# ai4co/rl4co

Hardware: AMD Instinct MI355X
Metric: decode_steps_per_sec (higher is better)
Workload: dtype bf16; 1 GPU; BASELINE configs[1]: TSPEnv num_loc=100 batch=4096/GPU AttentionModel(3L,d128,h8) greedy rollout, bf16 encoder GEMMs, bf16 cache; leg=c2_greedy, batch_per_gpu=4096, cache_dtype=bf16, launch=pipeline, input=one synthetic batch resident in HBM, reused by every step, parallelism=replicas x1 (instances sharded)

## Files before the change

### rl4co_amd/csrc/am_decode.hip

```cpp
#include <hip/hip_runtime.h>

#include "common.h"
#include "rl4co_math.h"

namespace {

constexpr int kD = RL4CO_EMBED_DIM;
constexpr int kH = RL4CO_NUM_HEADS;
constexpr int kDH = kD / kH;
constexpr int kUnroll = 4;
constexpr float kNegInf = -__builtin_huge_valf();
constexpr float kSqrtD = 11.3137084989847604f;

struct CacheF32 {
  using elem = float;
  using raw = float4;
  static constexpr int EPL = 4;
  __device__ static inline raw zero() { return make_float4(0.f, 0.f, 0.f, 0.f); }
  __device__ static inline raw ld(const elem* p) { return *reinterpret_cast<const float4*>(p); }
  __device__ static inline void cvt(const raw& t, float (&v)[4]) {
    v[0] = t.x; v[1] = t.y; v[2] = t.z; v[3] = t.w;
  }
};

// ... 146 lines not shown
      key = rl4co_expf(lp) / nz;
    }
    if (bc == 0x7fffffff || key > best) {
      best = key;
      bc = c;
    }
    if (a.entropy && lp > kNegInf) ent = fmaf(rl4co_expf(lp), lp, ent);
    if (alp) alp[j] = lp;
  }
  rl4co::bfly_argmax(best, bc);
  if (a.entropy) st.ent_acc = st.ent_acc - rl4co::bfly_sum<1, 64>(ent);
  wave_lds_sync();
  return commit_and_step<ENV>(a, st, lg, fl, F, mk, vis, dem, cap, r, t, N, lane, oplocs, opmax, twdur, bc);
}

template <int ENV>
__device__ inline int commit_and_step(const rl4co_am_decode_args& a, TrajState& st, float* lg, const uint16_t* fl, int F,
                                      uint8_t* mk, uint8_t* vis, const float* dem, float cap, int r, int t, int N, int lane,
                                      const float* oplocs, const float* opmax, const float* twdur, int bc) {
  const int64_t tcol = (int64_t)a.t0 + t;
  int bi;
  float logp;
  if (a.mode == RL4CO_DECODE_EVALUATE) {
    bi = (int)a.forced_actions[(int64_t)r * a.out_stride + tcol];
    if (bi < 0 || bi >= N) {
      st.errbits |= RL4CO_EBIT_INFEASIBLE;
      bi = 0;
    }
    int pos = 0x7fffffff;
    for (int c = lane; c < F; c += 64)
      if (fl[c] == bi) pos = c;
    pos = -rl4co::bfly_i_max(-pos);
    logp = pos < F ? lg[pos] : kNegInf;
  } else {
    bi = (bc < F) ? (int)fl[bc] : 0;
    logp = (bc < F) ? lg[bc] : kNegInf;
  }
  if (mk[bi] == 0) st.errbits |= RL4CO_EBIT_INFEASIBLE;
  if (!(logp > -1000.0f)) st.errbits |= RL4CO_EBIT_NEG_INF_LOGP;
  if (lane == 0) {
    a.actions[(int64_t)r * a.out_stride + tcol] = bi;
    a.logps[(int64_t)r * a.out_stride + tcol] = logp;
  }
  wave_lds_sync();

  if (ENV == RL4CO_ENV_TSP) {
    if (st.step_i == 0) st.first = bi;
    st.cur = bi;
    if (lane == 0) mk[bi] = 0;
    st.step_i += 1;
    wave_lds_sync();
    bool any_left = false;
    for (int j = lane; j < N; j += 64) any_left |= mk[j] != 0;
    st.done = !__any(any_left);
  } else if (ENV == RL4CO_ENV_PDP) {
    const int n = N - 1;
    if (lane == 0) {
      vis[bi] &= (uint8_t)~1u;
      vis[(bi + n / 2) % (n + 1)] |= 2;
    }
    st.step_i += 1;
    st.cur = bi;
    wave_lds_sync();
    bool left = false;
    for (int j = lane; j < N; j += 64) {
      const uint8_t v = vis[j];
      mk[j] = (v == 3) ? 1 : 0;
      left |= (v & 1) != 0;
    }
    st.done = !__any(left);
  } else if (ENV == RL4CO_ENV_PCTSP) {
    st.used = st.used + dem[bi];
    if (lane == 0) vis[bi] = 1;
    st.done = (bi == 0) && (st.step_i > 0);
    st.step_i += 1;
    st.cur = bi;
    wave_lds_sync();
    const bool depot_visited = vis[0] != 0;
    bool unvisited = false;
    for (int j = lane; j < N; j += 64) {
      if (j >= 1) {
        mk[j] = (vis[j] != 0 || depot_visited) ? 0 : 1;
        unvisited |= vis[j] == 0;
      }
    }
    unvisited = __any(unvisited);
    if (lane == 0) mk[0] = ((st.used < 1.0f) && unvisited) ? 0 : 1;
  } else if (ENV == RL4CO_ENV_OP) {
    const float cx = oplocs[2 * st.cur], cy = oplocs[2 * st.cur + 1];
    const float bx = oplocs[2 * bi], by = oplocs[2 * bi + 1];
    {
      const float dx = bx - cx, dy = by - cy;
      st.used = st.used + sqrtf(fmaf(dy, dy, dx * dx));
    }
    if (lane == 0) vis[bi] = 1;
    st.done = (bi == 0) && (st.step_i > 0);
    st.step_i += 1;
    st.cur = bi;
    wave_lds_sync();
    const bool depot_visited = vis[0] != 0;
    for (int j = lane; j < N; j += 64) {
      const float dx = oplocs[2 * j] - bx, dy = oplocs[2 * j + 1] - by;
      const bool exceeds = st.used + sqrtf(fmaf(dy, dy, dx * dx)) > opmax[j];
      mk[j] = (j == 0 || !(vis[j] != 0 || depot_visited || exceeds)) ? 1 : 0;
    }
  } else {
    if (ENV == RL4CO_ENV_CVRPTW) {
      const float dx = oplocs[2 * bi] - oplocs[2 * st.cur], dy = oplocs[2 * bi + 1] - oplocs[2 * st.cur + 1];
      const float served = fmaxf(st.time + sqrtf(fmaf(dy, dy, dx * dx)), opmax[2 * bi]) + twdur[bi];
      st.time = (bi != 0 ? 1.0f : 0.0f) * served;
    }
    const int di = min(max(bi - 1, 0), N - 2);
    st.used = (st.used + dem[di]) * (bi != 0 ? 1.0f : 0.0f);
    st.cur = bi;
    if (lane == 0) vis[bi] = 1;
    wave_lds_sync();
    const float thr = cap + 1e-5f;
    bool any_feasible = false, all_visited = true;
    for (int j = lane; j < N; j += 64) {
      all_visited &= vis[j] != 0;
      if (j >= 1) {
        const bool masked = (vis[j] != 0) || (dem[j - 1] + st.used > thr);
        mk[j] = masked ? 0 : 1;
        any_feasible |= !masked;
      }
    }
    any_feasible = __any(any_feasible);
    st.done = __all(all_visited);
    if (lane == 0) mk[0] = ((st.cur == 0) && any_feasible) ? 0 : 1;
    if (ENV == RL4CO_ENV_CVRPTW) {
      wave_lds_sync();
      const float bx = oplocs[2 * bi], by = oplocs[2 * bi + 1];
      for (int j = lane; j < N; j += 64) {
        const float dx = oplocs[2 * j] - bx, dy = oplocs[2 * j + 1] - by;
        if (!(st.time + sqrtf(fmaf(dy, dy, dx * dx)) <= opmax[2 * j + 1])) mk[j] = 0;
      }
    }
  }
  wave_lds_sync();
  return bi;
}

template <int EPL>
__device__ inline void gemv_t(float (&out)[EPL], const float* __restrict__ wt, const float* in_lds, int width, int e0) {
#pragma unroll
  for (int e = 0; e < EPL; ++e) out[e] = 0.0f;
  for (int k = 0; k < width; ++k) {
    const float c = in_lds[k];
#pragma unroll
    for (int e = 0; e < EPL; ++e) out[e] = fmaf(wt[(int64_t)k * kD + e0 + e], c, out[e]);
  }
}

template <class C, int ENV, bool UNFOLD = false>
__global__ void __launch_bounds__(64) am_decode_kernel(const rl4co_am_decode_args a) {
  constexpr int EPL = C::EPL;
  constexpr int LPR = kD / EPL;
  constexpr int RPL = 64 / LPR;
  constexpr int LPH = kDH / EPL;
  using elem = typename C::elem;
  using raw_t = typename C::raw;

  extern __shared__ __align__(16) unsigned char smem[];
  const int lane = threadIdx.x;
  const int r = trajectory_of_block(blockIdx.x, a.B, a.B_inst);
  const int N = a.N;
  const int Np = lds_pad(N);
  float* sc = reinterpret_cast<float*>(smem);
  float* lg = sc + Np * kH;
  float* mh = lg + Np;
  uint16_t* fl = reinterpret_cast<uint16_t*>(mh + kH);
  uint8_t* mk = reinterpret_cast<uint8_t*>(fl + Np);
  uint8_t* vis = mk + Np;

  const int cb = r % a.B_inst;
  const int rg = lane / LPR;
  const int li = lane % LPR;
  const int hd = li / LPH;
  const int e0 = li * EPL;

  const elem* Kg = static_cast<const elem*>(a.glimpse_key) + (int64_t)cb * a.kvl_batch_stride + e0;
  const elem* Vg = static_cast<const elem*>(a.glimpse_val) + (int64_t)cb * a.kvl_batch_stride + e0;
  const elem* Kl = static_cast<const elem*>(a.logit_key) + (int64_t)cb * a.kvl_batch_stride + e0;
  const int64_t rs = a.kvl_row_stride;
  const CtxTables<C> ctx(a, cb, N, e0);
  const float* hrow = UNFOLD ? a.node_embed + (int64_t)cb * N * kD + e0 : nullptr;

  uint8_t* gmask = a.action_mask + (int64_t)r * N;
  for (int j = lane; j < Np; j += 64) mk[j] = (j < N) ? gmask[j] : (uint8_t)0;
  constexpr bool kScalarCtx = ENV == RL4CO_ENV_CVRP || ENV == RL4CO_ENV_OP || ENV == RL4CO_ENV_PCTSP || ENV == RL4CO_ENV_CVRPTW;
  constexpr bool kCvrpLike = ENV == RL4CO_ENV_CVRP || ENV == RL4CO_ENV_CVRPTW;
  if (ENV == RL4CO_ENV_PDP) {
    const uint8_t* gv = a.visited + (int64_t)r * N;
    const uint8_t* gt = a.to_deliver + (int64_t)r * N;
    for (int j = lane; j < Np; j += 64) vis[j] = (j < N) ? (uint8_t)((gv[j] != 0 ? 1 : 0) | (gt[j] != 0 ? 2 : 0)) : (uint8_t)0;
  } else if (ENV != RL4CO_ENV_TSP) {
    const uint8_t* gv = a.visited + (int64_t)r * N;
    for (int j = lane; j < Np; j += 64) vis[j] = (j < N) ? gv[j] : (uint8_t)1;
  }
  TrajState st;
  st.cur = (int)a.current_node[r];
  st.first = (ENV == RL4CO_ENV_TSP) ? (int)a.first_node[r] : 0;
  st.step_i = !kCvrpLike ? a.step_i[r] : 0;
  st.time = (ENV == RL4CO_ENV_CVRPTW) ? a.current_time[r] : 0.0f;
  st.used = kScalarCtx ? a.used_capacity[r] : 0.0f;
  st.done = a.done[r] != 0;
  st.errbits = 0;
  st.ent_acc = 0.0f;
  const float* oplocs = (ENV == RL4CO_ENV_OP || ENV == RL4CO_ENV_CVRPTW) ? a.locs + (int64_t)cb * N * 2 : nullptr;
  const float* opmax = (ENV == RL4CO_ENV_OP)       ? a.max_length + (int64_t)cb * N
                       : (ENV == RL4CO_ENV_CVRPTW) ? a.time_windows + (int64_t)cb * N * 2
                                                   : nullptr;
  const float* twdur = (ENV == RL4CO_ENV_CVRPTW) ? a.durations + (int64_t)cb * N : nullptr;
  const float cap = (kCvrpLike || ENV == RL4CO_ENV_PCTSP) ? a.vehicle_capacity[r]
                                                                      : ((ENV == RL4CO_ENV_OP) ? opmax[0] : 0.0f);
  const float* dem = kCvrpLike                  ? a.demand + (int64_t)cb * (N - 1)
                     : (ENV == RL4CO_ENV_PCTSP) ? a.demand + (int64_t)cb * N
                                                : nullptr;
  wave_lds_sync();

  float qb[EPL];
#pragma unroll
  for (int e = 0; e < EPL; ++e) qb[e] = a.q_bias ? a.q_bias[(int64_t)cb * kD + e0 + e] : 0.0f;

  const bool single = a.max_steps == 1;
  int t = 0;
  int rows_read = 0;

  for (; t < a.max_steps && (!st.done || single); ++t) {
    const int F = build_list(a, mk, fl, N, lane);
    rows_read += F;

    float q[EPL];
    if constexpr (UNFOLD) {
      float* cv = sc;
      if (rg == 0) {
        if (ENV == RL4CO_ENV_TSP) {
          const bool ph = st.step_i < 1;
#pragma unroll
          for (int e = 0; e < EPL; ++e) {
            cv[e0 + e] = ph ? a.w_placeholder[e0 + e] : hrow[(int64_t)st.first * kD + e];
            cv[kD + e0 + e] = ph ? a.w_placeholder[kD + e0 + e] : hrow[(int64_t)st.cur * kD + e];
          }
        } else {
#pragma unroll
          for (int e = 0; e < EPL; ++e) cv[e0 + e] = hrow[(int64_t)st.cur * kD + e];
          if (li == 0) cv[kD] = cap - st.used;
        }
      }
      wave_lds_sync();
      gemv_t<EPL>(q, a.w_ctx_t, cv, a.ctx_width, e0);
#pragma unroll
      for (int e = 0; e < EPL; ++e) q[e] = q[e] + qb[e];
      wave_lds_sync();
    } else if (ENV == RL4CO_ENV_TSP) {
      if (st.step_i < 1) {
#pragma unroll
        for (int e = 0; e < EPL; ++e) q[e] = a.q_step0[e0 + e] + qb[e];
      } else {
        float cf[EPL], cc[EPL];
        ctx.load(ctx.first, st.first, cf);
        ctx.load(ctx.cur, st.cur, cc);
#pragma unroll
        for (int e = 0; e < EPL; ++e) q[e] = (cf[e] + cc[e]) + qb[e];
      }
    } else if (ENV == RL4CO_ENV_PDP) {
      float cc[EPL];
      ctx.load(ctx.cur, st.cur, cc);
#pragma unroll
      for (int e = 0; e < EPL; ++e) q[e] = cc[e] + qb[e];
    } else {
      float rem = cap - st.used;
      if (ENV == RL4CO_ENV_PCTSP && !(rem > 0.0f)) rem = 0.0f;
      float cc[EPL];
      ctx.load(ctx.cur, st.cur, cc);
#pragma unroll
      for (int e = 0; e < EPL; ++e) {
        float v = fmaf(a.w_cap[e0 + e], rem, cc[e]);
        if (ENV == RL4CO_ENV_CVRPTW) v = fmaf(a.w_time[e0 + e], st.time, v);
        q[e] = v + qb[e];
      }
    }
#pragma unroll
    for (int e = 0; e < EPL; ++e) q[e] = q[e] * 0.25f;

    float m = kNegInf;
    for (int c0 = 0; c0 < F; c0 += RPL * kUnroll) {
      raw_t rw[kUnroll];
      int jj[kUnroll];
#pragma unroll
      for (int u = 0; u < kUnroll; ++u) {
        const int c = c0 + u * RPL + rg;
        jj[u] = (c < F) ? (int)fl[c] : -1;
        rw[u] = (jj[u] >= 0) ? C::ld(Kg + (int64_t)jj[u] * rs) : C::zero();
      }
#pragma unroll
      for (int u = 0; u < kUnroll; ++u) {
        const int c = c0 + u * RPL + rg;
        const bool valid = jj[u] >= 0;
        float k[EPL];
        C::cvt(rw[u], k);
        float acc = 0.0f;
#pragma unroll
        for (int e = 0; e < EPL; ++e) acc = fmaf(q[e], k[e], acc);
        acc = rl4co::bfly_sum<1, LPH>(acc);
        const bool feas = valid && (!a.mask_inner || mk[valid ? jj[u] : 0] != 0);
        const float sv = feas ? acc : kNegInf;
        if (valid && (li % LPH) == 0) sc[c * kH + hd] = sv;
        m = fmaxf(m, sv);
      }
    }
    m = rl4co::bfly_max<LPR, 64>(m);
    if (rg == 0 && (li % LPH) == 0) mh[hd] = m;
    wave_lds_sync();
    {
      const float mm = mh[lane & (kH - 1)];
      for (int idx = lane; idx < F * kH; idx += 64) sc[idx] = rl4co_expf(sc[idx] - mm);
    }
    wave_lds_sync();

    float l = 0.0f;
    float o[EPL];
#pragma unroll
    for (int e = 0; e < EPL; ++e) o[e] = 0.0f;
    for (int c0 = 0; c0 < F; c0 += RPL * kUnroll) {
      raw_t rw[kUnroll];
      bool ok[kUnroll];
#pragma unroll
      for (int u = 0; u < kUnroll; ++u) {
        const int c = c0 + u * RPL + rg;
        ok[u] = c < F;
        rw[u] = ok[u] ? C::ld(Vg + (int64_t)fl[c] * rs) : C::zero();
      }
#pragma unroll
      for (int u = 0; u < kUnroll; ++u) {
        const int c = c0 + u * RPL + rg;
        float v[EPL];
        C::cvt(rw[u], v);
        const float p = ok[u] ? sc[c * kH + hd] : 0.0f;
        l = l + p;
#pragma unroll
        for (int e = 0; e < EPL; ++e) o[e] = fmaf(p, v[e], o[e]);
      }
    }
    l = 1.0f / rl4co::bfly_sum<LPR, 64>(l);
#pragma unroll
    for (int e = 0; e < EPL; ++e) o[e] = rl4co::bfly_sum<LPR, 64>(o[e]) * l;
    if constexpr (UNFOLD) {
      wave_lds_sync();
      if (rg == 0) {
#pragma unroll
        for (int e = 0; e < EPL; ++e) sc[e0 + e] = o[e];
      }
      wave_lds_sync();
      gemv_t<EPL>(o, a.w_out_t, sc, kD, e0);
    }

    for (int c0 = 0; c0 < F; c0 += RPL * kUnroll) {
      raw_t rw[kUnroll];
#pragma unroll
      for (int u = 0; u < kUnroll; ++u) {
        const int c = c0 + u * RPL + rg;
        rw[u] = (c < F) ? C::ld(Kl + (int64_t)fl[c] * rs) : C::zero();
      }
#pragma unroll
      for (int u = 0; u < kUnroll; ++u) {
        const int c = c0 + u * RPL + rg;
        float k[EPL];
        C::cvt(rw[u], k);
        float acc = 0.0f;
#pragma unroll
        for (int e = 0; e < EPL; ++e) acc = fmaf(o[e], k[e], acc);
        acc = rl4co::bfly_sum<1, LPR>(acc);
        if (c < F && li == 0) lg[c] = acc;
      }
    }
    wave_lds_sync();

    finalize_and_step<ENV>(a, st, lg, fl, F, mk, vis, dem, cap, r, t, N, lane, oplocs, opmax, twdur);
  }
  if (!single && !st.done && t >= a.max_steps) st.errbits |= RL4CO_EBIT_MAX_STEPS;

  for (int j = lane; j < N; j += 64) gmask[j] = mk[j];
  if (ENV == RL4CO_ENV_PDP) {
    uint8_t* gv = a.visited + (int64_t)r * N;
    uint8_t* gt = a.to_deliver + (int64_t)r * N;
    for (int j = lane; j < N; j += 64) {
      gv[j] = vis[j] & 1;
      gt[j] = (vis[j] >> 1) & 1;
    }
  } else if (ENV != RL4CO_ENV_TSP) {
    uint8_t* gv = a.visited + (int64_t)r * N;
    for (int j = lane; j < N; j += 64) gv[j] = vis[j];
  }
  if (lane == 0) {
    a.current_node[r] = st.cur;
    a.done[r] = st.done ? 1 : 0;
    if (ENV == RL4CO_ENV_TSP) a.first_node[r] = st.first;
    if (!kCvrpLike) a.step_i[r] = st.step_i;
    if (ENV == RL4CO_ENV_CVRPTW) a.current_time[r] = st.time;
    if (kScalarCtx) a.used_capacity[r] = st.used;
    if (a.n_steps) a.n_steps[r] = t;
    if (a.steps_summary) {
      atomicMax(a.steps_summary, t);
      atomicAdd(a.steps_summary + 1, t);
      atomicAdd(reinterpret_cast<unsigned long long*>(a.steps_summary + 2), (unsigned long long)rows_read);
    }
    if (a.entropy) a.entropy[r] += st.ent_acc;
    if (st.errbits) atomicOr(a.err, (int)st.errbits);
  }
}

constexpr int kLdsWaves = 4;
constexpr int kLdsGroups = 16;

template <int ENV>
__device__ inline int wide_scores(const rl4co_am_decode_args& a, TrajState& st, float* lg, const uint16_t* fl, int F,
                                  const uint8_t* mk, float* xs, int nw, int r, int t, int N, int tid) {
  constexpr int T = 64 * kLdsWaves;
  const int w = tid >> 6, lane = tid & 63;
  float* ex = xs;
  float* xw = xs + 2 * nw;
  bool nan_seen = false;
  float zmax = kNegInf;
  for (int c = tid; c < F; c += T) {
    float z = lg[c] / kSqrtD;
    if (z != z) nan_seen = true;
    if (a.tanh_clipping > 0.0f) z = rl4co_tanhf(z) * a.tanh_clipping;
    if (a.mask_logits && mk[fl[c]] == 0) z = kNegInf;
    if (a.temperature != 1.0f) z = z / a.temperature;
    lg[c] = z;
    zmax = fmaxf(zmax, z);
  }
  zmax = rl4co::bfly_max<1, 64>(zmax);
  const bool wave_nan = __any(nan_seen);
  if (lane == 0) {
    xw[w] = zmax;
    xw[4 + w] = wave_nan ? 1.0f : 0.0f;
  }
  __syncthreads();
  zmax = fmaxf(fmaxf(xw[0], xw[1]), fmaxf(xw[2], xw[3]));
  if ((xw[4] + xw[5]) + (xw[6] + xw[7]) != 0.0f) st.errbits |= RL4CO_EBIT_NAN_LOGIT;
  for (int c = tid; c < F; c += T) ex[c] = rl4co_expf(lg[c] - zmax);
  __syncthreads();
  if (w == 0) {
    float zsum = 0.0f;
    for (int c = lane; c < F; c += 64) zsum = zsum + ex[c];
    zsum = rl4co::bfly_sum<1, 64>(zsum);
    if (lane == 0) xw[8] = rl4co_logf(zsum);
  }
  __syncthreads();
  const float lse = xw[8];
  const int64_t tcol = (int64_t)a.t0 + t;
  float* alp = a.all_logps ? a.all_logps + ((int64_t)r * a.out_stride + tcol) * N : nullptr;
  if (alp && F < N) {
    for (int j = tid; j < N; j += T)
      if (mk[j] == 0) alp[j] = kNegInf;
  }
  for (int c = tid; c < F; c += T) {
    const int j = fl[c];
    const float lp = (lg[c] - zmax) - lse;
    lg[c] = lp;
    float key = lp;
    if (a.mode == RL4CO_DECODE_SAMPLE) {
      const float nz = a.exp_noise
                           ? a.exp_noise[((int64_t)t * a.B + r) * N + j]
                           : rl4co_exp1_noise(a.philox_seed ^ (a.philox_seed_dev ? *a.philox_seed_dev : 0ull),
                                              a.philox_offset + (uint64_t)tcol, (uint32_t)r,
                                              (uint32_t)j);
      key = rl4co_expf(lp) / nz;
    }
    ex[c] = key;
    if (alp) alp[j] = lp;
  }
  __syncthreads();
  int bc = 0x7fffffff;
  if (w == 0) {
    float best = kNegInf, ent = 0.0f;
    for (int c = lane; c < F; c += 64) {
      const float key = ex[c];
      if (bc == 0x7fffffff || key > best) {
        best = key;
        bc = c;
      }
      if (a.entropy) {
        const float lp = lg[c];
        if (lp > kNegInf) ent = fmaf(rl4co_expf(lp), lp, ent);
      }
    }
    rl4co::bfly_argmax(best, bc);
    if (a.entropy) st.ent_acc = st.ent_acc - rl4co::bfly_sum<1, 64>(ent);
    wave_lds_sync();
  }
  return bc;
}

__host__ __device__ inline int lds_variant_sc_rows(int N) { return N < 80 ? 80 : N; }
__host__ __device__ inline int wide_scratch_bytes(int N) {
  const int nw = (N + 3) & ~3;
  return lds_variant_sc_rows(N) * kH * 4 + nw * 4 + kLdsWaves * kH * 4 + 32 + 2 * nw + 2 * nw;
}
__host__ __device__ inline int lds_variant_bytes(int N) { return 3 * N * kD * 2 + wide_scratch_bytes(N); }

template <int ENV, bool RESIDENT, class C = CacheBF16>
__global__ void __launch_bounds__(64 * kLdsWaves, 4) am_decode_wide_kernel(const rl4co_am_decode_args a) {
  constexpr int EPL = 8, LPR = 16, LPH = 2;
  constexpr int U = 4;
  extern __shared__ __align__(16) unsigned char smem[];
  const int tid = threadIdx.x;
  const int w = tid >> 6, lane = tid & 63;
  const int r = trajectory_of_block(blockIdx.x, a.B, a.B_inst);
  const int N = a.N;
  const int nw = (N + 3) & ~3;
  uint16_t* planes = reinterpret_cast<uint16_t*>(smem);
  float* sc = reinterpret_cast<float*>(planes + (RESIDENT ? 3 * N * kD : 0));
  float* lg = sc + lds_variant_sc_rows(N) * kH;
  float* mpart = lg + nw;
  int* shi = reinterpret_cast<int*>(mpart + kLdsWaves * kH);
  uint16_t* fl = reinterpret_cast<uint16_t*>(shi + 8);
  uint8_t* mk = reinterpret_cast<uint8_t*>(fl + nw);
  uint8_t* vis = mk + nw;

  const int cb = r % a.B_inst;
  const int rg = lane / LPR, li = lane % LPR, hd = li / LPH, e0 = li * EPL;
  const uint16_t *Kg, *Vg, *Kl;
  int64_t rs;
  if constexpr (RESIDENT) {
    Kg = planes + e0;
    Vg = planes + N * kD + e0;
    Kl = planes + 2 * N * kD + e0;
    rs = kD;
  } else {
// ... 148 lines not shown
#pragma unroll
    for (int e = 0; e < EPL; ++e) o[e] = 0.0f;
    for (int i0 = 0; i0 < iters; i0 += U) {
      uint4 rw[U];
      bool ok[U];
#pragma unroll
      for (int u = 0; u < U; ++u) {
        const int c = kLdsGroups * (i0 + u) + 4 * w + rg;
        ok[u] = c < F;
        rw[u] = ok[u] ? *reinterpret_cast<const uint4*>(Vg + (int64_t)fl[c] * rs) : C::zero();
      }
#pragma unroll
      for (int u = 0; u < U; ++u) {
        const int c = kLdsGroups * (i0 + u) + 4 * w + rg;
        float v[EPL];
        C::cvt(rw[u], v);
        const float p = ok[u] ? sc[c * kH + hd] : 0.0f;
        l = l + p;
#pragma unroll
        for (int e = 0; e < EPL; ++e) o[e] = fmaf(p, v[e], o[e]);
      }
    }
    l = rl4co::bfly_sum<LPR, 64>(l);
#pragma unroll
    for (int e = 0; e < EPL; ++e) o[e] = rl4co::bfly_sum<LPR, 64>(o[e]);
    if (rg == 0) {
#pragma unroll
      for (int e = 0; e < EPL; ++e) *opart(w, e0 + e) = o[e];
      if ((li & 1) == 0) *lpart(w, hd) = l;
    }
    __syncthreads();
    l = 1.0f / ((*lpart(0, hd) + *lpart(1, hd)) + (*lpart(2, hd) + *lpart(3, hd)));
#pragma unroll
    for (int e = 0; e < EPL; ++e) {
      const int d = e0 + e;
      o[e] = ((*opart(0, d) + *opart(1, d)) + (*opart(2, d) + *opart(3, d))) * l;
    }

    for (int i0 = 0; i0 < iters; i0 += U) {
      uint4 rw[U];
#pragma unroll
      for (int u = 0; u < U; ++u) {
        const int c = kLdsGroups * (i0 + u) + 4 * w + rg;
        rw[u] = (c < F) ? *reinterpret_cast<const uint4*>(Kl + (int64_t)fl[c] * rs) : C::zero();
      }
#pragma unroll
      for (int u = 0; u < U; ++u) {
        const int c = kLdsGroups * (i0 + u) + 4 * w + rg;
        float k[EPL];
        C::cvt(rw[u], k);
        float acc = 0.0f;
#pragma unroll
        for (int e = 0; e < EPL; ++e) acc = fmaf(o[e], k[e], acc);
        acc = rl4co::bfly_sum<1, LPR>(acc);
        if (c < F && li == 0) lg[c] = acc;
      }
    }
    __syncthreads();

    const int bc = wide_scores<ENV>(a, st, lg, fl, F, mk, sc, nw, r, t, N, tid);
    if (w == 0) {
      commit_and_step<ENV>(a, st, lg, fl, F, mk, vis, dem, cap, r, t, N, lane, oplocs, opmax, twdur, bc);
      const int Fn = build_list(a, mk, fl, N, lane);
      if (lane == 0) {
        shi[0] = st.cur;
        shi[1] = st.done ? 1 : 0;
        shi[2] = Fn;
        shi[3] = st.first;
        shi[4] = (int)st.step_i;
        shi[5] = __float_as_int(st.used);
        shi[6] = __float_as_int(st.time);
      }
    }
    __syncthreads();
    if (w != 0) {
      st.cur = shi[0];
      st.done = shi[1] != 0;
      st.first = shi[3];
      st.step_i = shi[4];
      st.used = __int_as_float(shi[5]);
      st.time = __int_as_float(shi[6]);
    }
  }
  if (w == 0) {
    if (!single && !st.done && t >= a.max_steps) st.errbits |= RL4CO_EBIT_MAX_STEPS;
    for (int j = lane; j < N; j += 64) gmask[j] = mk[j];
    if (ENV == RL4CO_ENV_PDP) {
      uint8_t* gv = a.visited + (int64_t)r * N;
      uint8_t* gt = a.to_deliver + (int64_t)r * N;
      for (int j = lane; j < N; j += 64) {
        gv[j] = vis[j] & 1;
        gt[j] = (vis[j] >> 1) & 1;
      }
    } else if (ENV != RL4CO_ENV_TSP) {
      uint8_t* gv = a.visited + (int64_t)r * N;
      for (int j = lane; j < N; j += 64) gv[j] = vis[j];
    }
    if (lane == 0) {
      a.current_node[r] = st.cur;
      a.done[r] = st.done ? 1 : 0;
      if (ENV == RL4CO_ENV_TSP) a.first_node[r] = st.first;
      if (!kCvrpLike) a.step_i[r] = st.step_i;
      if (ENV == RL4CO_ENV_CVRPTW) a.current_time[r] = st.time;
      if (kScalarCtx) a.used_capacity[r] = st.used;
      if (a.n_steps) a.n_steps[r] = t;
      if (a.steps_summary) {
        atomicMax(a.steps_summary, t);
        atomicAdd(a.steps_summary + 1, t);
        atomicAdd(reinterpret_cast<unsigned long long*>(a.steps_summary + 2), (unsigned long long)(RESIDENT ? 0 : rows_read));
      }
      if (a.entropy) a.entropy[r] += st.ent_acc;
      if (st.errbits) atomicOr(a.err, (int)st.errbits);
    }
  }
}

template <int ENV, bool RESIDENT, class C>
int launch_wide_c(const rl4co_am_decode_args& a, hipStream_t stream) {
  const int lds = RESIDENT ? lds_variant_bytes(a.N) : wide_scratch_bytes(a.N);
  if (lds > 64 * 1024) {
    RL4CO_HIP_TRY(hipFuncSetAttribute(reinterpret_cast<const void*>(am_decode_wide_kernel<ENV, RESIDENT, C>),
                                      hipFuncAttributeMaxDynamicSharedMemorySize, lds));
  }
  hipLaunchKernelGGL((am_decode_wide_kernel<ENV, RESIDENT, C>), dim3(a.B), dim3(64 * kLdsWaves), lds, stream, a);
  RL4CO_HIP_TRY(hipGetLastError());
  return RL4CO_OK;
}
template <int ENV, bool RESIDENT>
int launch_wide(const rl4co_am_decode_args& a, hipStream_t stream) {
  return a.cache_dtype == RL4CO_DT_F16 ? launch_wide_c<ENV, RESIDENT, CacheF16>(a, stream)
                                       : launch_wide_c<ENV, RESIDENT, CacheBF16>(a, stream);
}

inline int resolve_variant(const rl4co_am_decode_args& a) {
  if (a.unfold) return (a.variant == RL4CO_VARIANT_AUTO || a.variant == RL4CO_VARIANT_STREAM) ? RL4CO_VARIANT_STREAM : -1;
  const bool f16 = a.cache_dtype == RL4CO_DT_F16;
  const bool bf16 = a.cache_dtype == RL4CO_DT_BF16 || f16;
  const bool ms_ok = bf16 && a.N <= 128 && a.B_inst > 0 && a.all_logps == nullptr && a.entropy == nullptr;
  if (a.variant == RL4CO_VARIANT_MS) return ms_ok ? RL4CO_VARIANT_MS : -1;
  const bool fits = bf16 && lds_variant_bytes(a.N) <= 80 * 1024;
  const bool wide_ok = bf16 && wide_scratch_bytes(a.N) <= 64 * 1024;
  if (a.variant == RL4CO_VARIANT_STREAM) return RL4CO_VARIANT_STREAM;
  if (a.variant == RL4CO_VARIANT_LDS) return fits ? RL4CO_VARIANT_LDS : -1;
  if (a.variant == RL4CO_VARIANT_WIDE) return wide_ok ? RL4CO_VARIANT_WIDE : -1;
  if (a.max_steps < 4) return RL4CO_VARIANT_STREAM;
  const int ms_from = (a.env == RL4CO_ENV_TSP || a.env == RL4CO_ENV_PDP || a.env == RL4CO_ENV_PCTSP) ? 3
                      : (a.env == RL4CO_ENV_CVRP ? 8 : 0);
  if (ms_ok && ms_from > 0 && a.B >= ms_from * a.B_inst) return RL4CO_VARIANT_MS;
  if (fits && a.B <= 1024) return RL4CO_VARIANT_LDS;
  if (wide_ok && a.B <= 2048) return RL4CO_VARIANT_WIDE;
  return RL4CO_VARIANT_STREAM;
}

template <class C, int ENV, bool UNFOLD = false>
int launch(const rl4co_am_decode_args& a, hipStream_t stream) {
  const int lds = rl4co_am_decode_lds_bytes(a.N, ENV);
  if (lds > 64 * 1024) {
    RL4CO_HIP_TRY(hipFuncSetAttribute(reinterpret_cast<const void*>(am_decode_kernel<C, ENV, UNFOLD>),
                                      hipFuncAttributeMaxDynamicSharedMemorySize, lds));
  }
  hipLaunchKernelGGL((am_decode_kernel<C, ENV, UNFOLD>), dim3(a.B), dim3(64), lds, stream, a);
  RL4CO_HIP_TRY(hipGetLastError());
  return RL4CO_OK;
}

}

extern "C" int rl4co_am_decode_lds_bytes(int N, int env) {
  (void)env;
  const int Np = lds_pad(N);
  return Np * kH * 4 + Np * 4 + kH * 4 + Np * 2 + Np + Np;
}

extern "C" int rl4co_am_decode_row_groups(const rl4co_am_decode_args* args) {
  if (args == nullptr) return -1;
  const int v = resolve_variant(*args);
  if (v < 0) return -1;
  if (v == RL4CO_VARIANT_MS) return 0;
  if (v == RL4CO_VARIANT_LDS || v == RL4CO_VARIANT_WIDE) return kLdsGroups;
  return args->cache_dtype != RL4CO_DT_F32 ? 64 / (kD / CacheBF16::EPL) : 64 / (kD / CacheF32::EPL);
}

extern "C" int rl4co_am_decode_variant(const rl4co_am_decode_args* args) {
  return args == nullptr ? -1 : resolve_variant(*args);
}

extern "C" int rl4co_am_decode(const rl4co_am_decode_args* args, void* stream) {
  RL4CO_REQUIRE(args != nullptr);
  const rl4co_am_decode_args& a = *args;
  RL4CO_REQUIRE(a.env == RL4CO_ENV_TSP || a.env == RL4CO_ENV_CVRP || a.env == RL4CO_ENV_OP ||
                a.env == RL4CO_ENV_PCTSP || a.env == RL4CO_ENV_PDP || a.env == RL4CO_ENV_CVRPTW);
  RL4CO_REQUIRE(a.B > 0 && a.B_inst > 0 && a.B % a.B_inst == 0);
  RL4CO_REQUIRE(a.N >= 2 && a.N <= 4096);
  RL4CO_REQUIRE(a.max_steps >= 1);
  RL4CO_REQUIRE(a.mode >= RL4CO_DECODE_GREEDY && a.mode <= RL4CO_DECODE_EVALUATE);
  RL4CO_REQUIRE(a.cache_dtype == RL4CO_DT_F32 || a.cache_dtype == RL4CO_DT_BF16 || a.cache_dtype == RL4CO_DT_F16);
  RL4CO_REQUIRE(a.cache_dtype != RL4CO_DT_F16 || !a.unfold);
  RL4CO_REQUIRE(a.glimpse_key && a.glimpse_val && a.logit_key && (a.ctx_cur || a.unfold));
  RL4CO_REQUIRE(a.unfold == 0 || a.unfold == 1);
  RL4CO_REQUIRE(a.ctx_dtype == RL4CO_DT_F32 || (a.ctx_dtype == a.cache_dtype && !a.unfold));
  RL4CO_REQUIRE(a.ctx_row_stride == 0 || (a.ctx_row_stride >= kD && a.ctx_row_stride % 8 == 0));
  RL4CO_REQUIRE(a.ctx_batch_stride == 0 || (a.ctx_batch_stride >= (int64_t)a.N * kD && a.ctx_batch_stride % 8 == 0));
  RL4CO_REQUIRE(a.ctx_dtype == RL4CO_DT_F32 || ((reinterpret_cast<uintptr_t>(a.ctx_cur) | reinterpret_cast<uintptr_t>(a.ctx_first)) & 15) == 0);
  if (a.unfold) {
    RL4CO_REQUIRE(a.env == RL4CO_ENV_TSP || a.env == RL4CO_ENV_CVRP);
    RL4CO_REQUIRE(a.node_embed && a.w_ctx_t && a.w_out_t);
    RL4CO_REQUIRE(a.ctx_width == (a.env == RL4CO_ENV_TSP ? 2 * kD : kD + 1));
    RL4CO_REQUIRE(a.env != RL4CO_ENV_TSP || a.w_placeholder);
  }
  RL4CO_REQUIRE(a.kvl_row_stride >= kD && a.kvl_row_stride % 8 == 0);
  RL4CO_REQUIRE(a.kvl_batch_stride >= (int64_t)a.N * kD && a.kvl_batch_stride % 8 == 0);
  RL4CO_REQUIRE(a.action_mask && a.current_node && a.done && a.actions && a.logps && a.err);
  RL4CO_REQUIRE(a.out_stride >= 1 && a.t0 >= 0 && (int64_t)a.t0 + a.max_steps <= a.out_stride);
  RL4CO_REQUIRE(a.temperature > 0.0f);
  RL4CO_REQUIRE((reinterpret_cast<uintptr_t>(a.steps_summary) & 7) == 0);
  RL4CO_REQUIRE(a.mode != RL4CO_DECODE_EVALUATE || a.forced_actions != nullptr);
  if (a.env == RL4CO_ENV_TSP) {
    RL4CO_REQUIRE(((a.ctx_first && a.q_step0) || a.unfold) && a.first_node && a.step_i);
  } else if (a.env == RL4CO_ENV_CVRP) {
    RL4CO_REQUIRE((a.w_cap || a.unfold) && a.demand && a.used_capacity && a.vehicle_capacity && a.visited);
  } else if (a.env == RL4CO_ENV_CVRPTW) {
    RL4CO_REQUIRE(a.w_cap && a.w_time && a.demand && a.used_capacity && a.vehicle_capacity && a.visited);
    RL4CO_REQUIRE(a.locs && a.time_windows && a.durations && a.current_time);
  } else if (a.env == RL4CO_ENV_PDP) {
    RL4CO_REQUIRE(a.visited && a.to_deliver && a.step_i && (a.N - 1) % 2 == 0);
  } else if (a.env == RL4CO_ENV_PCTSP) {
    RL4CO_REQUIRE(a.w_cap && a.demand && a.used_capacity && a.vehicle_capacity && a.step_i && a.visited);
  } else {
    RL4CO_REQUIRE(a.w_cap && a.locs && a.max_length && a.used_capacity && a.step_i && a.visited);
  }
  RL4CO_REQUIRE(rl4co_am_decode_lds_bytes(a.N, a.env) <= 160 * 1024);
  RL4CO_REQUIRE(a.variant >= RL4CO_VARIANT_AUTO && a.variant <= RL4CO_VARIANT_MS);
  const int variant = resolve_variant(a);
  RL4CO_REQUIRE(variant >= 0);
  hipStream_t s = rl4co::as_stream(stream);
  if (a.unfold) {
    if (a.cache_dtype == RL4CO_DT_F32)
      return a.env == RL4CO_ENV_TSP ? launch<CacheF32, RL4CO_ENV_TSP, true>(a, s) : launch<CacheF32, RL4CO_ENV_CVRP, true>(a, s);
    return a.env == RL4CO_ENV_TSP ? launch<CacheBF16, RL4CO_ENV_TSP, true>(a, s) : launch<CacheBF16, RL4CO_ENV_CVRP, true>(a, s);
  }
  if (variant == RL4CO_VARIANT_MS && a.cache_dtype == RL4CO_DT_F16) return rl4co::launch_decode_ms_f16(a, s);
  if (variant == RL4CO_VARIANT_MS) return rl4co::launch_decode_ms(a, s);
  if (variant == RL4CO_VARIANT_LDS || variant == RL4CO_VARIANT_WIDE) {
    const bool res = variant == RL4CO_VARIANT_LDS;
    switch (a.env) {
      case RL4CO_ENV_TSP: return res ? launch_wide<RL4CO_ENV_TSP, true>(a, s) : launch_wide<RL4CO_ENV_TSP, false>(a, s);
      case RL4CO_ENV_CVRP: return res ? launch_wide<RL4CO_ENV_CVRP, true>(a, s) : launch_wide<RL4CO_ENV_CVRP, false>(a, s);
      case RL4CO_ENV_OP: return res ? launch_wide<RL4CO_ENV_OP, true>(a, s) : launch_wide<RL4CO_ENV_OP, false>(a, s);
      case RL4CO_ENV_PCTSP: return res ? launch_wide<RL4CO_ENV_PCTSP, true>(a, s) : launch_wide<RL4CO_ENV_PCTSP, false>(a, s);
      case RL4CO_ENV_PDP: return res ? launch_wide<RL4CO_ENV_PDP, true>(a, s) : launch_wide<RL4CO_ENV_PDP, false>(a, s);
      default: return res ? launch_wide<RL4CO_ENV_CVRPTW, true>(a, s) : launch_wide<RL4CO_ENV_CVRPTW, false>(a, s);
    }
  }
  if (a.cache_dtype == RL4CO_DT_F16) {
    switch (a.env) {
      case RL4CO_ENV_TSP: return launch<CacheF16, RL4CO_ENV_TSP>(a, s);
      case RL4CO_ENV_CVRP: return launch<CacheF16, RL4CO_ENV_CVRP>(a, s);
      case RL4CO_ENV_OP: return launch<CacheF16, RL4CO_ENV_OP>(a, s);
      case RL4CO_ENV_PCTSP: return launch<CacheF16, RL4CO_ENV_PCTSP>(a, s);
      case RL4CO_ENV_PDP: return launch<CacheF16, RL4CO_ENV_PDP>(a, s);
      default: return launch<CacheF16, RL4CO_ENV_CVRPTW>(a, s);
    }
  }
  if (a.env == RL4CO_ENV_CVRPTW)
    return a.cache_dtype == RL4CO_DT_F32 ? launch<CacheF32, RL4CO_ENV_CVRPTW>(a, s)
                                         : launch<CacheBF16, RL4CO_ENV_CVRPTW>(a, s);
  if (a.env == RL4CO_ENV_PDP)
    return a.cache_dtype == RL4CO_DT_F32 ? launch<CacheF32, RL4CO_ENV_PDP>(a, s) : launch<CacheBF16, RL4CO_ENV_PDP>(a, s);
  if (a.env == RL4CO_ENV_PCTSP)
    return a.cache_dtype == RL4CO_DT_F32 ? launch<CacheF32, RL4CO_ENV_PCTSP>(a, s)
                                         : launch<CacheBF16, RL4CO_ENV_PCTSP>(a, s);
  if (a.env == RL4CO_ENV_OP)
    return a.cache_dtype == RL4CO_DT_F32 ? launch<CacheF32, RL4CO_ENV_OP>(a, s) : launch<CacheBF16, RL4CO_ENV_OP>(a, s);
  if (a.cache_dtype == RL4CO_DT_F32) {
    return a.env == RL4CO_ENV_TSP ? launch<CacheF32, RL4CO_ENV_TSP>(a, s)
                                  : launch<CacheF32, RL4CO_ENV_CVRP>(a, s);
  }
  return a.env == RL4CO_ENV_TSP ? launch<CacheBF16, RL4CO_ENV_TSP>(a, s)
                                : launch<CacheBF16, RL4CO_ENV_CVRP>(a, s);
}
```

Before: 131.6 million instance·step/s.

## Software-pipeline K/V/logit-key row loads across decode phases and set waves_per_eu

Restructures the three gather loops in the AM decode kernel so each loop issues the next block's row loads after computing the current block. The first block of the next phase (Kg→Vg→Kl) is loaded while the previous phase is still finishing, and for most envs the first Kg block is issued before the query is built. This hides global-memory latency behind compute and LDS syncs. It also adds an amdgpu_waves_per_eu(4) hint, which can limit registers; the extra live registers from prefetching could raise register pressure or cause spills.

```diff
diff --git a/rl4co_amd/csrc/am_decode.hip b/rl4co_amd/csrc/am_decode.hip
--- a/rl4co_amd/csrc/am_decode.hip
+++ b/rl4co_amd/csrc/am_decode.hip
@@ -323,7 +323,7 @@
 }
 
 template <class C, int ENV, bool UNFOLD = false>
-__global__ void __launch_bounds__(64) am_decode_kernel(const rl4co_am_decode_args a) {
+__global__ void __launch_bounds__(64) __attribute__((amdgpu_waves_per_eu(4))) am_decode_kernel(const rl4co_am_decode_args a) {
   constexpr int EPL = C::EPL;
   constexpr int LPR = kD / EPL;
   constexpr int RPL = 64 / LPR;
@@ -397,9 +397,22 @@
   int t = 0;
   int rows_read = 0;
 
+  constexpr int kBlk = RPL * kUnroll;
+  raw_t rw[kUnroll];
+  int F = 0;
+  auto load_block = [&](const elem* P, int c0) {
+#pragma unroll
+    for (int u = 0; u < kUnroll; ++u) {
+      const int c = c0 + u * RPL + rg;
+      rw[u] = (c < F) ? C::ld(P + (int64_t)fl[c] * rs) : C::zero();
+    }
+  };
+
   for (; t < a.max_steps && (!st.done || single); ++t) {
-    const int F = build_list(a, mk, fl, N, lane);
+    F = build_list(a, mk, fl, N, lane);
     rows_read += F;
+    constexpr bool kAhead = ENV != RL4CO_ENV_OP && ENV != RL4CO_ENV_CVRPTW;
+    if (kAhead) load_block(Kg, 0);
 
     float q[EPL];
     if constexpr (UNFOLD) {
@@ -453,31 +466,30 @@
     }
 #pragma unroll
     for (int e = 0; e < EPL; ++e) q[e] = q[e] * 0.25f;
+    if (!kAhead) load_block(Kg, 0);
 
     float m = kNegInf;
-    for (int c0 = 0; c0 < F; c0 += RPL * kUnroll) {
-      raw_t rw[kUnroll];
-      int jj[kUnroll];
+    for (int c0 = 0; c0 < F; c0 += kBlk) {
 #pragma unroll
       for (int u = 0; u < kUnroll; ++u) {
         const int c = c0 + u * RPL + rg;
-        jj[u] = (c < F) ? (int)fl[c] : -1;
-        rw[u] = (jj[u] >= 0) ? C::ld(Kg + (int64_t)jj[u] * rs) : C::zero();
-      }
-#pragma unroll
-      for (int u = 0; u < kUnroll; ++u) {
-        const int c = c0 + u * RPL + rg;
-        const bool valid = jj[u] >= 0;
+        const bool valid = c < F;
+        const int j = valid ? (int)fl[c] : 0;
         float k[EPL];
         C::cvt(rw[u], k);
         float acc = 0.0f;
 #pragma unroll
         for (int e = 0; e < EPL; ++e) acc = fmaf(q[e], k[e], acc);
         acc = rl4co::bfly_sum<1, LPH>(acc);
-        const bool feas = valid && (!a.mask_inner || mk[valid ? jj[u] : 0] != 0);
+        const bool feas = valid && (!a.mask_inner || mk[j] != 0);
         const float sv = feas ? acc : kNegInf;
         if (valid && (li % LPH) == 0) sc[c * kH + hd] = sv;
         m = fmaxf(m, sv);
+      }
+      if (c0 + kBlk < F) {
+        load_block(Kg, c0 + kBlk);
+      } else if (kAhead) {
+        load_block(Vg, 0);
       }
     }
     m = rl4co::bfly_max<LPR, 64>(m);
@@ -488,29 +500,27 @@
       for (int idx = lane; idx < F * kH; idx += 64) sc[idx] = rl4co_expf(sc[idx] - mm);
     }
     wave_lds_sync();
+    if (!kAhead) load_block(Vg, 0);
 
     float l = 0.0f;
     float o[EPL];
 #pragma unroll
     for (int e = 0; e < EPL; ++e) o[e] = 0.0f;
-    for (int c0 = 0; c0 < F; c0 += RPL * kUnroll) {
-      raw_t rw[kUnroll];
-      bool ok[kUnroll];
-#pragma unroll
-      for (int u = 0; u < kUnroll; ++u) {
-        const int c = c0 + u * RPL + rg;
-        ok[u] = c < F;
-        rw[u] = ok[u] ? C::ld(Vg + (int64_t)fl[c] * rs) : C::zero();
-      }
+    for (int c0 = 0; c0 < F; c0 += kBlk) {
 #pragma unroll
       for (int u = 0; u < kUnroll; ++u) {
         const int c = c0 + u * RPL + rg;
         float v[EPL];
         C::cvt(rw[u], v);
-        const float p = ok[u] ? sc[c * kH + hd] : 0.0f;
+        const float p = (c < F) ? sc[c * kH + hd] : 0.0f;
         l = l + p;
 #pragma unroll
         for (int e = 0; e < EPL; ++e) o[e] = fmaf(p, v[e], o[e]);
+      }
+      if (c0 + kBlk < F) {
+        load_block(Vg, c0 + kBlk);
+      } else if (kAhead && !UNFOLD) {
+        load_block(Kl, 0);
       }
     }
     l = 1.0f / rl4co::bfly_sum<LPR, 64>(l);
@@ -525,14 +535,9 @@
       wave_lds_sync();
       gemv_t<EPL>(o, a.w_out_t, sc, kD, e0);
     }
-
-    for (int c0 = 0; c0 < F; c0 += RPL * kUnroll) {
-      raw_t rw[kUnroll];
-#pragma unroll
-      for (int u = 0; u < kUnroll; ++u) {
-        const int c = c0 + u * RPL + rg;
-        rw[u] = (c < F) ? C::ld(Kl + (int64_t)fl[c] * rs) : C::zero();
-      }
+    if (UNFOLD || !kAhead) load_block(Kl, 0);
+
+    for (int c0 = 0; c0 < F; c0 += kBlk) {
 #pragma unroll
       for (int u = 0; u < kUnroll; ++u) {
         const int c = c0 + u * RPL + rg;
@@ -544,6 +549,7 @@
         acc = rl4co::bfly_sum<1, LPR>(acc);
         if (c < F && li == 0) lg[c] = acc;
       }
+      if (c0 + kBlk < F) load_block(Kl, c0 + kBlk);
     }
     wave_lds_sync();
 
```

After: 131.0 million instance·step/s (median of 2 runs). About the same (-0.5%).

## Cache a few candidate K/V/logit-key rows in spare LDS for the stream decode

Applied to the files above, without the earlier changes.

Adds a small per-workgroup LDS row cache for TSP and CVRP in the stream decode kernel. Cached candidates are taken from the tail of the feasible list. The three cache planes (glimpse key, glimpse value, logit key) are filled on first read, and later steps read from LDS instead of HBM. When a node leaves the candidate set its slot passes to the next candidate. The slot count is sized on the host so it never lowers workgroups per CU. The aim is less HBM gather traffic per step, at the cost of extra per-step bookkeeping, wave reductions and LDS syncs, for what may be only a handful of cached rows.

```diff
diff --git a/rl4co_amd/csrc/am_decode.hip b/rl4co_amd/csrc/am_decode.hip
--- a/rl4co_amd/csrc/am_decode.hip
+++ b/rl4co_amd/csrc/am_decode.hip
@@ -322,12 +322,18 @@
   }
 }
 
+constexpr int kRowCacheNone = 0xFF;
+__host__ __device__ inline int row_cache_bytes(int N, int S, int esz) {
+  return S > 0 ? S * 3 * kD * esz + lds_pad(N) + S : 0;
+}
+
 template <class C, int ENV, bool UNFOLD = false>
-__global__ void __launch_bounds__(64) am_decode_kernel(const rl4co_am_decode_args a) {
+__global__ void __launch_bounds__(64) am_decode_kernel(const rl4co_am_decode_args a, const int S) {
   constexpr int EPL = C::EPL;
   constexpr int LPR = kD / EPL;
   constexpr int RPL = 64 / LPR;
   constexpr int LPH = kDH / EPL;
+  constexpr bool kRowCache = !UNFOLD && (ENV == RL4CO_ENV_TSP || ENV == RL4CO_ENV_CVRP);
   using elem = typename C::elem;
   using raw_t = typename C::raw;
 
@@ -342,6 +348,9 @@
   uint16_t* fl = reinterpret_cast<uint16_t*>(mh + kH);
   uint8_t* mk = reinterpret_cast<uint8_t*>(fl + Np);
   uint8_t* vis = mk + Np;
+  elem* rc = reinterpret_cast<elem*>(vis + Np);
+  uint8_t* rslot = reinterpret_cast<uint8_t*>(rc + S * 3 * kD);
+  uint8_t* rpend = rslot + Np;
 
   const int cb = r % a.B_inst;
   const int rg = lane / LPR;
@@ -389,6 +398,34 @@
                                                 : nullptr;
   wave_lds_sync();
 
+  const bool list_all = !(a.mask_inner && a.mask_logits);
+  auto candidate = [&](int j) -> bool {
+    return list_all || (ENV == RL4CO_ENV_TSP ? mk[j] != 0 : (j == 0 || vis[j] == 0));
+  };
+  const bool caching = kRowCache && S > 0;
+  if (caching) {
+    for (int j = lane; j < Np; j += 64) rslot[j] = (uint8_t)kRowCacheNone;
+    wave_lds_sync();
+    int k = 0;
+    for (int j0 = N - 1; j0 >= 0 && k < S; j0 -= 64) {
+      const int j = j0 - lane;
+      const bool f = j >= 0 && candidate(j);
+      const unsigned long long bal = __ballot(f);
+      const int s = k + __popcll(bal & ((1ull << lane) - 1ull));
+      if (f && s < S) {
+        rslot[j] = (uint8_t)s;
+        rpend[s] = 1;
+      }
+      k += __popcll(bal);
+    }
+    wave_lds_sync();
+  }
+  auto lds_row = [&](int j, int plane) -> const elem* { return rc + (rslot[j] * 3 + plane) * kD + e0; };
+  auto fill_row = [&](int j, int plane, const raw_t& v) {
+    const int s = rslot[j];
+    if (s != kRowCacheNone) *reinterpret_cast<raw_t*>(rc + (s * 3 + plane) * kD + e0) = v;
+  };
+
   float qb[EPL];
 #pragma unroll
   for (int e = 0; e < EPL; ++e) qb[e] = a.q_bias ? a.q_bias[(int64_t)cb * kD + e0 + e] : 0.0f;
@@ -399,7 +436,20 @@
 
   for (; t < a.max_steps && (!st.done || single); ++t) {
     const int F = build_list(a, mk, fl, N, lane);
-    rows_read += F;
+    int hend = F, pbeg = F;
+    if (caching) {
+      const int c_lo = max(F - S, 0);
+      int last_hbm = c_lo - 1, first_pend = F;
+      for (int c = c_lo + lane; c < F; c += 64) {
+        const int s = rslot[fl[c]];
+        const bool pend = s != kRowCacheNone && rpend[s] != 0;
+        if (s == kRowCacheNone || pend) last_hbm = c;
+        if (pend) first_pend = min(first_pend, c);
+      }
+      hend = rl4co::bfly_i_max(last_hbm) + 1;
+      pbeg = -rl4co::bfly_i_max(-first_pend);
+    }
+    rows_read += hend;
 
     float q[EPL];
     if constexpr (UNFOLD) {
@@ -455,6 +505,19 @@
     for (int e = 0; e < EPL; ++e) q[e] = q[e] * 0.25f;
 
     float m = kNegInf;
+    auto score = [&](const raw_t& rw, int c, int j) {
+      const bool valid = j >= 0;
+      float k[EPL];
+      C::cvt(rw, k);
+      float acc = 0.0f;
+#pragma unroll
+      for (int e = 0; e < EPL; ++e) acc = fmaf(q[e], k[e], acc);
+      acc = rl4co::bfly_sum<1, LPH>(acc);
+      const bool feas = valid && (!a.mask_inner || mk[valid ? j : 0] != 0);
+      const float sv = feas ? acc : kNegInf;
+      if (valid && (li % LPH) == 0) sc[c * kH + hd] = sv;
+      m = fmaxf(m, sv);
+    };
     for (int c0 = 0; c0 < F; c0 += RPL * kUnroll) {
       raw_t rw[kUnroll];
       int jj[kUnroll];
@@ -462,22 +525,13 @@
       for (int u = 0; u < kUnroll; ++u) {
         const int c = c0 + u * RPL + rg;
         jj[u] = (c < F) ? (int)fl[c] : -1;
-        rw[u] = (jj[u] >= 0) ? C::ld(Kg + (int64_t)jj[u] * rs) : C::zero();
+        rw[u] = (jj[u] < 0) ? C::zero() : (c < hend ? C::ld(Kg + (int64_t)jj[u] * rs) : C::ld(lds_row(jj[u], 0)));
       }
 #pragma unroll
       for (int u = 0; u < kUnroll; ++u) {
         const int c = c0 + u * RPL + rg;
-        const bool valid = jj[u] >= 0;
-        float k[EPL];
-        C::cvt(rw[u], k);
-        float acc = 0.0f;
-#pragma unroll
-        for (int e = 0; e < EPL; ++e) acc = fmaf(q[e], k[e], acc);
-        acc = rl4co::bfly_sum<1, LPH>(acc);
-        const bool feas = valid && (!a.mask_inner || mk[valid ? jj[u] : 0] != 0);
-        const float sv = feas ? acc : kNegInf;
-        if (valid && (li % LPH) == 0) sc[c * kH + hd] = sv;
-        m = fmaxf(m, sv);
+        if (caching && c >= pbeg && c < hend) fill_row(jj[u], 0, rw[u]);
+        score(rw[u], c, jj[u]);
       }
     }
     m = rl4co::bfly_max<LPR, 64>(m);
@@ -493,6 +547,14 @@
     float o[EPL];
 #pragma unroll
     for (int e = 0; e < EPL; ++e) o[e] = 0.0f;
+    auto accumulate = [&](const raw_t& rw, int c, bool ok) {
+      float v[EPL];
+      C::cvt(rw, v);
+      const float p = ok ? sc[c * kH + hd] : 0.0f;
+      l = l + p;
+#pragma unroll
+      for (int e = 0; e < EPL; ++e) o[e] = fmaf(p, v[e], o[e]);
+    };
     for (int c0 = 0; c0 < F; c0 += RPL * kUnroll) {
       raw_t rw[kUnroll];
       bool ok[kUnroll];
@@ -500,17 +562,13 @@
       for (int u = 0; u < kUnroll; ++u) {
         const int c = c0 + u * RPL + rg;
         ok[u] = c < F;
-        rw[u] = ok[u] ? C::ld(Vg + (int64_t)fl[c] * rs) : C::zero();
+        rw[u] = !ok[u] ? C::zero() : (c < hend ? C::ld(Vg + (int64_t)fl[c] * rs) : C::ld(lds_row(fl[c], 1)));
       }
 #pragma unroll
       for (int u = 0; u < kUnroll; ++u) {
         const int c = c0 + u * RPL + rg;
-        float v[EPL];
-        C::cvt(rw[u], v);
-        const float p = ok[u] ? sc[c * kH + hd] : 0.0f;
-        l = l + p;
-#pragma unroll
-        for (int e = 0; e < EPL; ++e) o[e] = fmaf(p, v[e], o[e]);
+        if (caching && c >= pbeg && c < hend) fill_row(fl[c], 1, rw[u]);
+        accumulate(rw[u], c, ok[u]);
       }
     }
     l = 1.0f / rl4co::bfly_sum<LPR, 64>(l);
@@ -526,28 +584,54 @@
       gemv_t<EPL>(o, a.w_out_t, sc, kD, e0);
     }
 
+    auto logit = [&](const raw_t& rw, int c) {
+      float k[EPL];
+      C::cvt(rw, k);
+      float acc = 0.0f;
+#pragma unroll
+      for (int e = 0; e < EPL; ++e) acc = fmaf(o[e], k[e], acc);
+      acc = rl4co::bfly_sum<1, LPR>(acc);
+      if (c < F && li == 0) lg[c] = acc;
+    };
     for (int c0 = 0; c0 < F; c0 += RPL * kUnroll) {
       raw_t rw[kUnroll];
 #pragma unroll
       for (int u = 0; u < kUnroll; ++u) {
         const int c = c0 + u * RPL + rg;
-        rw[u] = (c < F) ? C::ld(Kl + (int64_t)fl[c] * rs) : C::zero();
+        rw[u] = (c >= F) ? C::zero() : (c < hend ? C::ld(Kl + (int64_t)fl[c] * rs) : C::ld(lds_row(fl[c], 2)));
       }
 #pragma unroll
       for (int u = 0; u < kUnroll; ++u) {
         const int c = c0 + u * RPL + rg;
-        float k[EPL];
-        C::cvt(rw[u], k);
-        float acc = 0.0f;
-#pragma unroll
-        for (int e = 0; e < EPL; ++e) acc = fmaf(o[e], k[e], acc);
-        acc = rl4co::bfly_sum<1, LPR>(acc);
-        if (c < F && li == 0) lg[c] = acc;
+        if (caching && c >= pbeg && c < hend) fill_row(fl[c], 2, rw[u]);
+        logit(rw[u], c);
+      }
+    }
+    if (caching) {
+      for (int c = pbeg + lane; c < hend; c += 64) {
+        const int s = rslot[fl[c]];
+        if (s != kRowCacheNone) rpend[s] = 0;
       }
     }
     wave_lds_sync();
 
-    finalize_and_step<ENV>(a, st, lg, fl, F, mk, vis, dem, cap, r, t, N, lane, oplocs, opmax, twdur);
+    const int bi = finalize_and_step<ENV>(a, st, lg, fl, F, mk, vis, dem, cap, r, t, N, lane, oplocs, opmax, twdur);
+    if (caching && rslot[bi] != kRowCacheNone && !candidate(bi)) {
+      int nxt = -1;
+      for (int j = lane; j < N; j += 64)
+        if (candidate(j) && rslot[j] == kRowCacheNone) nxt = j;
+      nxt = rl4co::bfly_i_max(nxt);
+      const int s = rslot[bi];
+      wave_lds_sync();
+      if (lane == 0) {
+        rslot[bi] = (uint8_t)kRowCacheNone;
+        if (nxt >= 0) {
+          rslot[nxt] = (uint8_t)s;
+          rpend[s] = 1;
+        }
+      }
+      wave_lds_sync();
+    }
   }
   if (!single && !st.done && t >= a.max_steps) st.errbits |= RL4CO_EBIT_MAX_STEPS;
 
@@ -1002,14 +1086,38 @@
   return RL4CO_VARIANT_STREAM;
 }
 
+constexpr int kStreamWgPerCu = 16;
+constexpr int kCuLds = 160 * 1024;
+inline int stream_wg_per_cu(int bytes, int gran) {
+  const int b = (bytes + gran - 1) / gran * gran;
+  return min(kStreamWgPerCu, kCuLds / b);
+}
+
+int row_cache_slots(const rl4co_am_decode_args& a, int esz, bool unfold) {
+  if (unfold || a.max_steps == 1 || (a.env != RL4CO_ENV_TSP && a.env != RL4CO_ENV_CVRP)) return 0;
+  const int base = rl4co_am_decode_lds_bytes(a.N, a.env);
+  int S = 0;
+  while (S < min(a.N, 255)) {
+    const int bytes = base + row_cache_bytes(a.N, S + 1, esz);
+    if (stream_wg_per_cu(bytes, 512) < stream_wg_per_cu(base, 512) ||
+        stream_wg_per_cu(bytes, 1280) < stream_wg_per_cu(base, 1280) || bytes > kCuLds)
+      break;
+    ++S;
+  }
+  const char* e = getenv("RL4CO_DECODE_ROW_CACHE");
+  if (e && e[0] != '\0') return min(S, max(atoi(e), 0));
+  return esz == 4 ? 0 : S;
+}
+
 template <class C, int ENV, bool UNFOLD = false>
 int launch(const rl4co_am_decode_args& a, hipStream_t stream) {
-  const int lds = rl4co_am_decode_lds_bytes(a.N, ENV);
+  const int S = row_cache_slots(a, (int)sizeof(typename C::elem), UNFOLD);
+  const int lds = rl4co_am_decode_lds_bytes(a.N, ENV) + row_cache_bytes(a.N, S, (int)sizeof(typename C::elem));
   if (lds > 64 * 1024) {
     RL4CO_HIP_TRY(hipFuncSetAttribute(reinterpret_cast<const void*>(am_decode_kernel<C, ENV, UNFOLD>),
                                       hipFuncAttributeMaxDynamicSharedMemorySize, lds));
   }
-  hipLaunchKernelGGL((am_decode_kernel<C, ENV, UNFOLD>), dim3(a.B), dim3(64), lds, stream, a);
+  hipLaunchKernelGGL((am_decode_kernel<C, ENV, UNFOLD>), dim3(a.B), dim3(64), lds, stream, a, S);
   RL4CO_HIP_TRY(hipGetLastError());
   return RL4CO_OK;
 }
```

Measured after the change: 130.1 million instance·step/s before, 141.0 million instance·step/s after (median of 6 runs). 8.4% higher.
